# WenjieWWJ/FoodRec

Measured on NVIDIA B200. Metric: bpr_train_triples_per_sec, higher is better.
Workload: dtype f32

## Files before the change

foodrec_b200/csrc/api.cu:

```cuda
#include "ctx.h"

extern "C" int fr_abi_version(void) { return FR_ABI_VERSION; }

extern "C" int fr_create(const fr_config* cfg, fr_handle* out) {
  if (!cfg || !out) return FR_ERR_ARG;
  *out = nullptr;
  fr_ctx* h = new fr_ctx();
  *out = h;
  h->cfg = *cfg;
  const int D = cfg->embed_size;
  if (D <= 0 || D % 4 != 0 || D > 256) return fail(h, FR_ERR_ARG, "embed_size must be a multiple of 4 in (0,256], got %d", D);
  if (cfg->num_users <= 0 || cfg->num_items <= 0 || cfg->num_labels <= 0 || cfg->max_rows <= 0)
    return fail(h, FR_ERR_ARG, "num_users/num_items/num_labels/max_rows must be positive");
  if (cfg->learner < FR_SGD || cfg->learner > FR_ADAM) return fail(h, FR_ERR_ARG, "bad learner %d", cfg->learner);
  if (cfg->learner == FR_ADAM && cfg->adam_mode == FR_ADAM_LAZY_SERIES) {
    const double b1 = cfg->adam_beta1, b2 = cfg->adam_beta2;
    if (!(b1 >= 0.0 && b1 < 1.0 && b2 > 0.0 && b2 < 1.0)) return fail(h, FR_ERR_ARG, "adam betas must lie in [0,1) / (0,1)");
    double lead = 0.0, rem = 0.0, p1 = 1.0;
    for (int j = 1; j <= SERIES_WINDOW; ++j) {
      p1 *= b1;
      const double d = 1.0 - pow(b2, 0.5 * j);
      lead += p1;
      rem += p1 * pow(d, SERIES_TERMS) / (1.0 - d);
    }
// ... 1 lines not shown
      return fail(h, FR_ERR_UNSUPPORTED, "adam_mode LAZY_SERIES does not cover beta1=%g beta2=%g (tail %.1e, truncation %.1e): "
                  "use FR_ADAM_LAZY_EXACT", b1, b2, p1, lead > 0.0 ? rem / lead : 0.0);
  }
  int ndev = 0;
  cudaError_t e = cudaGetDeviceCount(&ndev);
  if (e != cudaSuccess || ndev == 0)
    return fail(h, FR_ERR_CUDA, "no CUDA device (%s); foodrec_b200 has no CPU fallback", cudaGetErrorString(e));
  FR_CUDA(h, cudaGetDevice(&h->device));
  cudaDeviceProp prop;
  FR_CUDA(h, cudaGetDeviceProperties(&prop, h->device));
  h->sm_count = prop.multiProcessorCount;
  h->l2_persist_max = (size_t)prop.persistingL2CacheMaxSize;
  h->l2_window_max = (size_t)prop.accessPolicyMaxWindowSize;
  if (getenv("FOODREC_NO_L2_PIN")) h->l2_persist_max = 0;
  if (getenv("FOODREC_DEBUG_L2"))
    fprintf(stderr, "foodrec_b200: L2 %d MB, persisting max %zu MB, access window max %zu MB\n", prop.l2CacheSize >> 20,
            h->l2_persist_max >> 20, h->l2_window_max >> 20);
  h->mc.D = D; h->mc.DV = D / 4; h->mc.L = cfg->num_labels;
  h->mc.a = cfg->high_level_score_coefficient;
  h->mc.oma = 1.0f - cfg->high_level_score_coefficient;
  h->mc.beta_1 = cfg->beta_1; h->mc.beta_2 = cfg->beta_2; h->mc.alpha = cfg->alpha;
  h->NV = h->mc.DV <= 32 ? 1 : 2;
  h->b1p = cfg->adam_beta1; h->b2p = cfg->adam_beta2;

  const size_t S = (size_t)cfg->max_rows, E = (size_t)(cfg->max_label_entries > 0 ? cfg->max_label_entries : 1);
  const size_t DV = h->mc.DV;
  int rc;
#define A(p, n) if ((rc = dalloc(h, &(p), (n)))) return rc
  A(h->ukeys, S); A(h->users_s, S); A(h->items_s, S); A(h->ws_row, S); A(h->g, S); A(h->scores, S); A(h->z, S * DV);
  if ((rc = alloc_sort(h, h->sortU, S))) return rc;
  if ((rc = alloc_sort(h, h->sortI, S))) return rc;
  if ((rc = alloc_sort(h, h->sortL, E))) return rc;
  h->fwd_grid_cap = h->sm_count * 4;
  A(h->part_loss, h->fwd_grid_cap); A(h->part_nrm, h->fwd_grid_cap); A(h->part_gcat, (size_t)h->fwd_grid_cap * 4 * DV);
  A(h->packed, 4 + 4 * (size_t)D + 5 * (size_t)cfg->num_labels * D);
  const size_t chS = S / 32 + 2, chE = E / 32 + 2;
  A(h->pieces_u, chS * 2 * 5 * DV); A(h->pieces_i, chS * 2 * DV); A(h->pieces_g, chE * 2 * 5 * DV);
  h->long_cap = (uint32_t)((chS > chE ? chS : chE) / FR_LONG_CHAIN + 2);
  A(h->long_list, h->long_cap);
  A(h->counts, S + 1); A(h->offs, S + 1); A(h->ent_key, E); A(h->ent_row, E); A(h->ent_coef, E); A(h->n_entries, 1);
  A(h->counters, 4); A(h->cat_pre, 4 * DV); A(h->mean_partials, 1024); A(h->out_internal, FR_OUT_COUNT);
  A(h->scan_tmp, S / 4096 + 2);
  h->lr_hist_cap = 1 << 16;
  A(h->lr_hist, (size_t)h->lr_hist_cap);
  A(h->cser, (size_t)h->lr_hist_cap * SERIES_TERMS);
#undef A
  FR_CUDA(h, cudaMemset(h->lr_hist, 0, (size_t)h->lr_hist_cap * sizeof(float)));
  FR_CUDA(h, cudaMemset(h->cser, 0, (size_t)h->lr_hist_cap * SERIES_TERMS * sizeof(double)));
  FR_CUDA(h, cudaMemset(h->out_internal, 0, FR_OUT_COUNT * sizeof(float)));
  return FR_OK;
}

extern "C" int64_t fr_launch_count(void) { return (int64_t)fr::g_launches; }

bool l2_window(fr_ctx* h, const void* ptr, size_t bytes, cudaAccessPolicyWindow* w) {
  if (!h->l2_persist_max || !h->l2_window_max || !bytes) return false;
  static bool limit_set = false;
  if (!limit_set) { cudaDeviceSetLimit(cudaLimitPersistingL2CacheSize, h->l2_persist_max); cudaGetLastError(); limit_set = true; }
  const size_t win = bytes < h->l2_window_max ? bytes : h->l2_window_max;
  w->base_ptr = const_cast<void*>(ptr);
  w->num_bytes = win;
  const double r = (double)h->l2_persist_max / (double)win;
  w->hitRatio = r >= 1.0 ? 1.0f : (float)r;
  w->hitProp = cudaAccessPropertyPersisting;
  w->missProp = cudaAccessPropertyNormal;
  return true;
}

extern "C" int fr_timing_enable(fr_handle h, int32_t enable) {
  if (!h) return FR_ERR_ARG;
  if (enable && h->tsets.empty()) {
    h->tsets.resize(32);
    for (auto& ts : h->tsets)
      for (auto& e : ts.ev) FR_CUDA(h, cudaEventCreate(&e));
  }
  h->timing = enable != 0;
  return FR_OK;
}

extern "C" int fr_timing_read(fr_handle h, double* ms_sum, int64_t* n_steps, int32_t reset) {
  if (!h || !ms_sum || !n_steps) return FR_ERR_ARG;
  for (auto& ts : h->tsets) timing_collect(h, ts);
  for (int i = 0; i < FR_T_COUNT; ++i) ms_sum[i] = h->t_sum[i];
  *n_steps = h->t_steps;
  if (reset) { for (auto& x : h->t_sum) x = 0.0; h->t_steps = 0; }
  return FR_OK;
}

extern "C" int fr_destroy(fr_handle h) {
  if (!h) return FR_OK;
  for (auto& ts : h->tsets) for (auto& e : ts.ev) cudaEventDestroy(e);
  catalog_free(h);
  for (void* p : h->allocs) cudaFree(p);
  if (h->stage) cudaFree(h->stage);
  for (auto& sl : h->feed) { if (sl.buf) cudaFree(sl.buf); if (sl.copied) cudaEventDestroy(sl.copied); if (sl.consumed) cudaEventDestroy(sl.consumed); }
  if (h->copy_stream) cudaStreamDestroy(h->copy_stream);
  if (h->aux_stream) { cudaStreamDestroy(h->aux_stream); cudaEventDestroy(h->aux_fork); cudaEventDestroy(h->aux_fork2); cudaEventDestroy(h->aux_join);
                       cudaStreamDestroy(h->aux2_stream); cudaEventDestroy(h->aux2_fork); cudaEventDestroy(h->aux2_join); }
  if (h->pieces_personal) cudaFree(h->pieces_personal);
  delete h;
  return FR_OK;
}

extern "C" const char* fr_last_error(fr_handle h) { return h ? h->err : "null handle"; }

extern "C" int fr_set_tables(fr_handle h, const fr_tables* t) {
// ... 551 lines not shown
```

foodrec_b200/csrc/common.cuh:

```cuda
#pragma once
#include <cuda_bf16.h>
#include <cuda_runtime.h>
#include <stdint.h>

#define FR_FULL 0xffffffffu
#define FR_WARPS_PER_BLOCK 8
#define FR_THREADS (FR_WARPS_PER_BLOCK * 32)

namespace fr {

__device__ __forceinline__ float warp_sum(float v) {
#pragma unroll
  for (int o = 16; o; o >>= 1) v += __shfl_xor_sync(FR_FULL, v, o);
  return v;
}
__device__ __forceinline__ double warp_sum_d(double v) {
#pragma unroll
  for (int o = 16; o; o >>= 1) v += __shfl_xor_sync(FR_FULL, v, o);
  return v;
}
__device__ __forceinline__ float4 f4zero() { return make_float4(0.f, 0.f, 0.f, 0.f); }
__device__ __forceinline__ float dot4(const float4 a, const float4 b) {
  return fmaf(a.w, b.w, fmaf(a.z, b.z, fmaf(a.y, b.y, a.x * b.x)));
}
__device__ __forceinline__ void fma4(float4& acc, const float s, const float4 v) {
  acc.x = fmaf(s, v.x, acc.x); acc.y = fmaf(s, v.y, acc.y);
  acc.z = fmaf(s, v.z, acc.z); acc.w = fmaf(s, v.w, acc.w);
}
__device__ __forceinline__ void mad4_rn(float4& acc, const float s, const float4 v) {
  acc.x = __fadd_rn(acc.x, __fmul_rn(s, v.x)); acc.y = __fadd_rn(acc.y, __fmul_rn(s, v.y));
  acc.z = __fadd_rn(acc.z, __fmul_rn(s, v.z)); acc.w = __fadd_rn(acc.w, __fmul_rn(s, v.w));
}
__device__ __forceinline__ float4 div4_rn(const float4 v, const float n) {
  return make_float4(__fdiv_rn(v.x, n), __fdiv_rn(v.y, n), __fdiv_rn(v.z, n), __fdiv_rn(v.w, n));
}
__device__ __forceinline__ float4 add4(const float4 a, const float4 b) {
  return make_float4(a.x + b.x, a.y + b.y, a.z + b.z, a.w + b.w);
}
__device__ __forceinline__ float4 scale4(const float s, const float4 v) {
  return make_float4(s * v.x, s * v.y, s * v.z, s * v.w);
}
__device__ __forceinline__ float4 shfl4(const float4 v, const int src) {
  return make_float4(__shfl_sync(FR_FULL, v.x, src), __shfl_sync(FR_FULL, v.y, src),
                     __shfl_sync(FR_FULL, v.z, src), __shfl_sync(FR_FULL, v.w, src));
}

__device__ __forceinline__ float4 ld_stream(const float4* p) {
  float4 r;
  asm volatile("ld.global.L1::no_allocate.v4.f32 {%0,%1,%2,%3}, [%4];"
               : "=f"(r.x), "=f"(r.y), "=f"(r.z), "=f"(r.w) : "l"(p));
  return r;
}
__device__ __forceinline__ void st_stream(float4* p, const float4 v) {
  asm volatile("st.global.L1::no_allocate.v4.f32 [%0], {%1,%2,%3,%4};"
               :: "l"(p), "f"(v.x), "f"(v.y), "f"(v.z), "f"(v.w) : "memory");
}

__device__ __forceinline__ void prefetch_l2_warp(const void* p, uint32_t bytes, int lane) {
#if defined(FR_PREFETCH_LINES)
  for (uint32_t o = (uint32_t)lane * 128u; o < bytes; o += 32u * 128u)
    asm volatile("prefetch.global.L2 [%0];" :: "l"(reinterpret_cast<const char*>(p) + o));
#else
  if (lane == 0) asm volatile("cp.async.bulk.prefetch.L2.global [%0], %1;" :: "l"(p), "r"(bytes) : "memory");
#endif
}

template <int NV>
__device__ __forceinline__ void load_row(float4 (&dst)[NV], const float4* row, int DV, int lane) {
#pragma unroll
  for (int k = 0; k < NV; ++k) {
    const int i = lane + 32 * k;
    dst[k] = (i < DV) ? ld_stream(row + i) : f4zero();
  }
}
template <int NV>
__device__ __forceinline__ void load_row_ro(float4 (&dst)[NV], const float4* __restrict__ row, int DV, int lane) {
#pragma unroll
  for (int k = 0; k < NV; ++k) {
    const int i = lane + 32 * k;
    dst[k] = (i < DV) ? __ldg(row + i) : f4zero();
  }
}
template <int NV>
__device__ __forceinline__ void load_row_cs(float4 (&dst)[NV], const float4* row, int DV, int lane) {
#pragma unroll
  for (int k = 0; k < NV; ++k) {
    const int i = lane + 32 * k;
    dst[k] = (i < DV) ? __ldcs(row + i) : f4zero();
  }
}
template <int NV>
__device__ __forceinline__ void store_row(float4* row, const float4 (&src)[NV], int DV, int lane) {
#pragma unroll
  for (int k = 0; k < NV; ++k) {
    const int i = lane + 32 * k;
    if (i < DV) st_stream(row + i, src[k]);
  }
}

template <bool BF> struct TabVec { using type = float4; };
template <> struct TabVec<true> { using type = uint2; };
template <bool BF>
__device__ __forceinline__ const typename TabVec<BF>::type* tab_at(const float4* base, size_t idx4) {
  return reinterpret_cast<const typename TabVec<BF>::type*>(base) + idx4;
}
template <bool BF>
__device__ __forceinline__ typename TabVec<BF>::type* tab_at(float4* base, size_t idx4) {
  return reinterpret_cast<typename TabVec<BF>::type*>(base) + idx4;
}
__device__ __forceinline__ float4 bf4_to_f4(const uint2 v) {
  return make_float4(__uint_as_float(v.x << 16), __uint_as_float(v.x & 0xffff0000u),
                     __uint_as_float(v.y << 16), __uint_as_float(v.y & 0xffff0000u));
}
__device__ __forceinline__ uint2 f4_to_bf4(const float4 v) {
  const __nv_bfloat162 a = __floats2bfloat162_rn(v.x, v.y), b = __floats2bfloat162_rn(v.z, v.w);
  uint2 r;
  r.x = *reinterpret_cast<const uint32_t*>(&a); r.y = *reinterpret_cast<const uint32_t*>(&b);
  return r;
// ... 97 lines not shown
```

foodrec_b200/csrc/eval.cu:

```cuda
#include "common.cuh"
#include "internal.h"

namespace fr {

template <int NV, class V>
__device__ __forceinline__ float score_pair(const float4 (&pr)[5][NV], const V* __restrict__ Rrow,
                                            const float4 m, const float4* sCat, int DV, int lane,
                                            float a, float oma) {
  float4 rr[NV], pcs[NV];
  load_row_ro_t<NV>(rr, Rrow, DV, lane);
  pooled_cat<NV>(pcs, sCat, m, DV, lane);
  float hs = 0.f, ls = 0.f;
#pragma unroll
  for (int k = 0; k < NV; ++k) {
    float4 zs;
    zs.x = m.x * pr[1][k].x + m.y * pr[2][k].x + m.z * pr[3][k].x + m.w * pr[4][k].x;
    zs.y = m.x * pr[1][k].y + m.y * pr[2][k].y + m.z * pr[3][k].y + m.w * pr[4][k].y;
    zs.z = m.x * pr[1][k].z + m.y * pr[2][k].z + m.z * pr[3][k].z + m.w * pr[4][k].z;
    zs.w = m.x * pr[1][k].w + m.y * pr[2][k].w + m.z * pr[3][k].w + m.w * pr[4][k].w;
    hs += dot4(pr[0][k], pcs[k]);
    ls += dot4(zs, rr[k]);
  }
  hs = warp_sum(hs); ls = warp_sum(ls);
  const float n = ((m.x + m.y) + m.z) + m.w;
// ... 3 lines not shown
template <int NV, bool BF>
__global__ void __launch_bounds__(FR_THREADS)
fwd_score_kernel(const float4* __restrict__ P, const float4* __restrict__ R, const float4* __restrict__ Cat,
                 int DV, const int32_t* __restrict__ users, const int32_t* __restrict__ items,
                 const float4* __restrict__ cats, int cats_by_item, int n, float a, float oma,
                 float* __restrict__ scores, const HealthBlend hb, uint32_t n_users, uint32_t n_items) {
  extern __shared__ float4 sCat[];
  for (int i = threadIdx.x; i < 4 * DV; i += blockDim.x) sCat[i] = Cat[i];
  __syncthreads();
  const int lane = threadIdx.x & 31;
  const int gw = blockIdx.x * FR_WARPS_PER_BLOCK + (threadIdx.x >> 5), nw = gridDim.x * FR_WARPS_PER_BLOCK;
  int cur_u = -1;
  float4 pr[5][NV];
  constexpr int RPW = 8;
  for (int blk = gw; blk * RPW < n; blk += nw) {
    for (int q = 0; q < RPW; ++q) {
      const int r = blk * RPW + q;
      if (r >= n) break;
      const int u = users[r];
      const int it = items[r];
      if ((uint32_t)u >= n_users || (uint32_t)it >= n_items) {
        if (lane == 0) scores[r] = __int_as_float(0x7fc00000);
        continue;
      }
      if (u != cur_u) {
#pragma unroll
        for (int s = 0; s < 5; ++s) load_row_ro_t<NV>(pr[s], tab_at<BF>(P, ((size_t)u * 5 + s) * DV), DV, lane);
        health_blend_rows<NV>(pr, hb, u, DV, lane);
        cur_u = u;
      }
      const float4 m = __ldg(cats + (cats_by_item ? it : r));
      const float s = score_pair<NV>(pr, tab_at<BF>(R, (size_t)it * DV), m, sCat, DV, lane, a, oma);
      if (lane == 0) scores[r] = s;
    }
  }
}

void launch_fwd_score(const ModelConsts& mc, const float4* P, const float4* R, const float4* Cat,
                      const int32_t* users, const int32_t* items, const float4* cats,
                      int cats_by_item, int n, float* scores, const HealthBlend& hb, const Launch& l,
                      int64_t n_users, int64_t n_items, int bf16) {
  if (n <= 0) return;
  int grid = (n + 8 * FR_WARPS_PER_BLOCK - 1) / (8 * FR_WARPS_PER_BLOCK);
  if (grid > l.sm_count * 8) grid = l.sm_count * 8;
  const size_t smem = (size_t)4 * mc.DV * sizeof(float4);
  ++g_launches;
#define FR_SCORE(NVV, BFF) fwd_score_kernel<NVV, BFF><<<grid, FR_THREADS, smem, l.st>>>(P, R, Cat, mc.DV, users, items, cats, cats_by_item, \
    n, mc.a, mc.oma, scores, hb, (uint32_t)n_users, (uint32_t)n_items)
  if (mc.DV <= 32) { if (bf16) FR_SCORE(1, true); else FR_SCORE(1, false); }
  else             { if (bf16) FR_SCORE(2, true); else FR_SCORE(2, false); }
#undef FR_SCORE
}

__device__ __forceinline__ void cp_async_vec(float4* dst, const float4* src) {
  const uint32_t d = (uint32_t)__cvta_generic_to_shared(dst);
  asm volatile("cp.async.cg.shared.global [%0], [%1], 16;" :: "r"(d), "l"(src) : "memory");
}
__device__ __forceinline__ void cp_async_vec(uint2* dst, const uint2* src) {
  const uint32_t d = (uint32_t)__cvta_generic_to_shared(dst);
  asm volatile("cp.async.ca.shared.global [%0], [%1], 8;" :: "r"(d), "l"(src) : "memory");
}
__device__ __forceinline__ void cp_async_commit() { asm volatile("cp.async.commit_group;" ::: "memory"); }
template <int N> __device__ __forceinline__ void cp_async_wait() { asm volatile("cp.async.wait_group %0;" :: "n"(N) : "memory"); }
__device__ __forceinline__ float4 ring_ld(const float4* p) { return *p; }
__device__ __forceinline__ float4 ring_ld(const uint2* p) { return bf4_to_f4(*p); }

constexpr int EV_WARPS = 4;
constexpr int EV_THREADS = EV_WARPS * 32;
constexpr int EV_CB = 8;
#ifndef FR_EV_GROUPS
#define FR_EV_GROUPS 2
#endif
#ifndef FR_EV_MINB
#define FR_EV_MINB 4
#endif
template <int NV> struct EvRing { static constexpr int GROUPS = FR_EV_GROUPS; };

template <int NV, int SLOTS, bool BF, bool EXACT>
__global__ void __launch_bounds__(EV_THREADS, NV == 1 ? FR_EV_MINB : (FR_EV_MINB > 3 ? 3 : FR_EV_MINB))
eval_sampled_kernel(const float4* __restrict__ P, const float4* __restrict__ R, const float4* __restrict__ Cat,
                    int DV, float a, float oma, const int32_t* __restrict__ users,
                    const int32_t* __restrict__ cand, const int32_t* __restrict__ n_cand, int n_users,
                    int stride, const float4* __restrict__ cand_cats, const float4* __restrict__ item_cats,
                    int K, int32_t* __restrict__ topk_ids, int32_t* __restrict__ gt_rank,
                    float* __restrict__ scores_out, const HealthBlend hb, uint32_t n_table_users, uint32_t n_items) {
  extern __shared__ float4 smem[];
  float4* sCat = smem;
  for (int i = threadIdx.x; i < 4 * DV; i += blockDim.x) sCat[i] = Cat[i];
  __syncthreads();
  const int lane = threadIdx.x & 31;
  float4* sM = smem + 4 * DV + (threadIdx.x >> 5) * (40 * SLOTS);
  uint32_t* sO = reinterpret_cast<uint32_t*>(sM + 32 * SLOTS);
  using V = typename TabVec<BF>::type;
  constexpr int GROUPS = EvRing<NV>::GROUPS;
  V* const ring = reinterpret_cast<V*>(smem + 4 * DV + EV_WARPS * (40 * SLOTS)) + ((threadIdx.x >> 5) * (GROUPS * EV_CB * NV) * 32 + lane);
  const int gw = blockIdx.x * EV_WARPS + (threadIdx.x >> 5), nw = gridDim.x * EV_WARPS;
  const typename TabVec<BF>::type* Rl = tab_at<BF>(R, 0) + lane;
  asm volatile("" : "+l"(Rl));
  constexpr int VB = (int)sizeof(typename TabVec<BF>::type);
  int un = 0, ncn = 0, idn[SLOTS];
  float4 pr[5][NV], mqn[SLOTS];
  auto fetch_ids = [&](int w2) {
    if (w2 < n_users) {
      un = users[w2]; ncn = n_cand[w2];
#pragma unroll
      for (int q = 0; q < SLOTS; ++q) {
        const int j = q * 32 + lane;
        idn[q] = j < stride ? cand[(size_t)w2 * stride + j] : -1;
      }
    }
  };
  auto fetch_rows = [&](int w2) {
    if (w2 >= n_users) return;
    if ((uint32_t)un < n_table_users) {
#pragma unroll
      for (int s = 0; s < 5; ++s) load_row_cs_t<NV>(pr[s], tab_at<BF>(P, ((size_t)un * 5 + s) * DV), DV, lane);
// ... 235 lines not shown
```

foodrec_b200/csrc/train.cuh:

```cuda
#pragma once
#include "internal.h"

namespace fr {

struct FwdParams {
  const float4 *P, *R, *cat;
  int DV, B;
  float Bnorm;
  const int32_t *users, *items;
  const float4* cats; int cats_by_item;
  const float* labels;
  float a, oma;
  float* g; float4* z; float* scores;
  float *part_loss, *part_nrm; float4* part_gcat;
  int lazy; const float4 *mP, *vP; const int32_t* lastP; OptConsts oc;
  int tab;
};

struct FinalizeParams {
  const float *part_loss, *part_nrm; const float4* part_gcat; int nblk;
  int DV; float inv_count_B;
  float B;
  float* packed;
  int do_reduce, do_apply;
  float4 *Cat, *s1Cat, *s2Cat;
  OptConsts oc; float clip;
  float* out; float* lr_hist;
};

struct SegCommon {
  const uint32_t* keys; const uint32_t* perm;
  const uint32_t* n_dev; uint32_t n_host;
  float4* pieces;
  uint32_t* uniq_counter;
  uint4* long_list;
  uint32_t* long_count; uint32_t long_cap;
  const float* only_if_scaled;
};
constexpr uint32_t FR_LONG_CHAIN = 16;

struct UserPolParams {
  float4 *P, *s1, *s2; int32_t* last;
  const float4 *R, *G; const float4* cat;
  const int32_t* items; const float* g; const float4* cats; int cats_by_item;
  const float* ws_row; const float* out;
  int group; ModelConsts mc; OptConsts oc;
  const float* user_labels; const int32_t *lab_off, *lab_idx; const int32_t* users;
  int tab;
};
struct FusedParams {
  float4 *P[2], *m[2], *v[2];
  int32_t* last;
  const float4 *R, *cat;
  const int32_t* items; const float4* cats; int cats_by_item;
  const float* labels;
  float a, oma, Bnorm;
  float* g; float4* z; float* scores;
  float *part_loss, *part_nrm; float4* part_gcat;
  ModelConsts mc; OptConsts oc;
};
int user_fused_grid(uint32_t n_rows, int sm_count);
void launch_user_fused(int NV, int group, const SegCommon& c, const FusedParams& p, int grid, const Launch& l);
void launch_user_commit(const uint32_t* keys, uint32_t n, int32_t* last, const float* out, int step, const Launch& l);
void launch_shadow_consolidate(int32_t* last, int64_t n_users, int rowDV, float4* P, float4* m, float4* v, const float4* Pa,
                               const float4* ma, const float4* va, const float* pred, const Launch& l);

struct ItemPolParams {
  float4 *R, *s1, *s2; int32_t* last;
  const float4* z; const float* g; const float* out;
  ModelConsts mc; OptConsts oc;
  int tab;
};
struct LabelPolParams {
  float4* G; const float4 *R, *cat;
  const uint32_t* ent_row; const float* ent_coef;
  const int32_t* items; const float4* cats; int cats_by_item;
  ModelConsts mc;
  int tab;
};

struct LabelEmitParams {
  int S, group, L; const int32_t* users;
  const float* user_labels; const int32_t *lab_off, *lab_idx;
  const float* ws_row;
  uint32_t* counts;
  const uint32_t* offs;
  uint32_t *ent_key, *ent_row; float* ent_coef; uint32_t cap;
  uint32_t* n_entries; float* out;
};

void launch_prep_rows(int mode, int B, const int32_t* users, const int32_t* items, const float* labels, const float* ws_in,
                      int64_t n_users, int64_t n_items, uint32_t* ukeys, float* ws_row, int32_t* users_s, int32_t* items_s,
                      float* flag, const Launch& l);
void launch_fwd_train(int NV, int group, const FwdParams& p, int grid, const Launch& l);
int fwd_train_grid(int B, int sm_count);
void launch_finalize(const FinalizeParams& p, const Launch& l);
void launch_user_pass(int NV, const SegCommon& c, const UserPolParams& p, const Launch& l);
void launch_personal_pass(int NV, const SegCommon& c, const UserPolParams& p, const Launch& l);
void launch_item_pass(int NV, const SegCommon& c, const ItemPolParams& p, const Launch& l);
void launch_label_pass(int NV, const SegCommon& c, const LabelPolParams& p, const Launch& l);
void launch_label_count(const LabelEmitParams& p, const Launch& l);
void launch_label_emit(const LabelEmitParams& p, const Launch& l);
void launch_adam_sweep(float4* var, float4* m, float4* v, int32_t* last, int64_t nrows, int rowDV,
                       const OptConsts& oc, int target_step, const Launch& l);
void launch_fill_i32(int32_t* p, int64_t n, int32_t v, const Launch& l);
void launch_series_update(double* cser, const float* lr_hist, int t, float b1, float b2, const Launch& l);
void launch_series_rebuild(double* cser, const float* lr_hist, int step, float b1, float b2, const Launch& l);
void launch_item_catchup(int NV, const uint32_t* keys, uint32_t n, float4* R, float4* m, float4* v,
                         int32_t* last, int DV, const OptConsts& oc, const Launch& l,
                         const uint32_t* n_dev = nullptr);
struct PeerPtrs { float4* dst[8]; int world, rank, cap; };
void launch_item_grad_pass(int NV, const SegCommon& c, const ItemPolParams& p, float4* gbuf, const PeerPtrs& peers, const Launch& l);

struct ShardPlanParams {
// ... 32 lines not shown
```

foodrec_b200/csrc/train_seg.cu:

```cuda
#include <cstdlib>

#include "optim.cuh"
#include "train.cuh"

namespace fr {

template <class Pol>
__global__ void __launch_bounds__(FR_THREADS)
seg_chunk_kernel(const SegCommon c, const Pol pol) {
  extern __shared__ float4 smem[];
  constexpr int NR = Pol::NR, NV = Pol::NV;
  const int DV = pol.DV();
  if (c.only_if_scaled && c.only_if_scaled[FR_OUT_SCALE] == 1.0f) return;
  if (pol.cat_src()) {
    for (int i = threadIdx.x; i < 4 * DV; i += blockDim.x) smem[i] = pol.cat_src()[i];
    __syncthreads();
  }
  const uint32_t n = c.n_dev ? min(*c.n_dev, c.n_host) : c.n_host;
  const uint32_t nchunks = (n + 31) >> 5;
  const int lane = threadIdx.x & 31;
  const uint32_t gw = blockIdx.x * FR_WARPS_PER_BLOCK + (threadIdx.x >> 5);
  const uint32_t nw = gridDim.x * FR_WARPS_PER_BLOCK;
  for (uint32_t chunk = gw; chunk < nchunks; chunk += nw) {
    const uint32_t base = chunk << 5;
// ... 740 lines not shown
  if (l.mid) cudaEventRecord(l.mid, l.st);
  seg_combine_kernel<Pol><<<grid, FR_THREADS, 0, l.st>>>(c, pol);
  g_launches += 2;
  launch_combine_long(c, pol, DV, l);
}

template <int NVV, int OPT>
struct FusedUserPol {
  static constexpr int NV = NVV;
  static constexpr int NR = 5;
  FusedParams p;
  struct State { float4 var[5][NVV], s1[5][NVV], s2[5][NVV]; int last, sh; };
  __device__ __forceinline__ int DV() const { return p.mc.DV; }
  __device__ __forceinline__ void load_state(State& st, uint32_t key, int lane) const {
    const int l = p.last[key];
    st.sh = (l >> 30) & 1; st.last = l & 0x3fffffff;
    const int DVv = p.mc.DV;
    const size_t base = (size_t)key * 5 * DVv;
    const float4 *Ps = p.P[st.sh] + base, *ms = p.m[st.sh] + base, *vs = p.v[st.sh] + base;
#pragma unroll
    for (int s = 0; s < 5; ++s)
#pragma unroll
      for (int k = 0; k < NV; ++k) {
        const int i = lane + 32 * k;
        const bool ok = i < DVv;
        st.var[s][k] = ok ? __ldcs(Ps + s * DVv + i) : f4zero();
        st.s1[s][k] = ok ? __ldcs(ms + s * DVv + i) : f4zero();
        st.s2[s][k] = ok ? __ldcs(vs + s * DVv + i) : f4zero();
      }
  }
  __device__ __forceinline__ void apply_to_other(State& st, uint32_t key, const float4 (&grad)[5][NV], int lane, bool caught) const {
    if (!caught) adam_catchup<OPT, 5 * NV>(&st.var[0][0], &st.s1[0][0], &st.s2[0][0], st.last, p.oc.step - 1, p.oc);
    const int DVv = p.mc.DV;
    const size_t base = (size_t)key * 5 * DVv;
    float4 *Pd = p.P[st.sh ^ 1] + base, *md = p.m[st.sh ^ 1] + base, *vd = p.v[st.sh ^ 1] + base;
#pragma unroll
    for (int s = 0; s < 5; ++s)
#pragma unroll
      for (int k = 0; k < NV; ++k) {
        const int i = lane + 32 * k;
        if (i >= DVv) continue;
        float4 var = st.var[s][k], a = st.s1[s][k], b = st.s2[s][k];
        const float4 g = grad[s][k];
        adam_touch(var.x, a.x, b.x, g.x, p.oc); adam_touch(var.y, a.y, b.y, g.y, p.oc);
        adam_touch(var.z, a.z, b.z, g.z, p.oc); adam_touch(var.w, a.w, b.w, g.w, p.oc);
        __stcs(Pd + s * DVv + i, var); __stcs(md + s * DVv + i, a); __stcs(vd + s * DVv + i, b);
      }
  }
  __device__ __forceinline__ void apply(State& st, uint32_t key, float4 (&acc)[5][NV], int lane) const {
    apply_to_other(st, key, acc, lane, false);
  }
};

template <int NV, int GROUP, int OPT>
__global__ void __launch_bounds__(FR_THREADS, NV == 1 ? 2 : 1)
user_fused_kernel(const SegCommon c, const FusedUserPol<NV, OPT> pol) {
  extern __shared__ float4 smem[];
  const FusedParams& p = pol.p;
  const int DV = p.mc.DV;
  float4* sCat = smem;
  float4* sgc = smem + 4 * DV;
  __shared__ float red_loss[FR_WARPS_PER_BLOCK], red_nrm[FR_WARPS_PER_BLOCK];
  for (int i = threadIdx.x; i < 4 * DV; i += blockDim.x) sCat[i] = p.cat[i];
  for (int i = threadIdx.x; i < FR_WARPS_PER_BLOCK * 4 * DV; i += blockDim.x) sgc[i] = f4zero();
  __syncthreads();
  const int lane = threadIdx.x & 31, warp = threadIdx.x >> 5;
  float4* mygc = sgc + warp * 4 * DV;
  const uint32_t n = c.n_host;
  const uint32_t nchunks = (n + 31) >> 5;
  const uint32_t gw = blockIdx.x * FR_WARPS_PER_BLOCK + warp, nw = gridDim.x * FR_WARPS_PER_BLOCK;
  const float a = p.a, oma = p.oma, Bf = p.Bnorm;
  float lossacc = 0.f, nrmacc = 0.f;
  for (uint32_t chunk = gw; chunk < nchunks; chunk += nw) {
    const uint32_t base = chunk << 5;
    const int cnt = (int)min(32u, n - base);
    const bool valid = lane < cnt;
    const uint32_t key = valid ? c.keys[base + lane] : 0xffffffffu;
    const uint32_t ent = valid ? c.perm[base + lane] : 0u;
    const uint32_t prevKey = base > 0 ? c.keys[base - 1] : 0u;
    const bool has_next = base + 32 < n;
    const uint32_t nextKey = has_next ? c.keys[base + 32] : 0u;
    int e_item = 0; float4 e_m = make_float4(1.f, 0.f, 0.f, 0.f); float e_y = 0.f; int e_last = 0;
    if (valid) {
      e_item = p.items[ent];
      e_m = __ldg(p.cats + (p.cats_by_item ? e_item : (int)ent));
      if (GROUP == 1) e_y = p.labels[ent];
      e_last = p.last[key];
    }
    const uint32_t up = __shfl_up_sync(FR_FULL, key, 1);
    const bool head = valid && (lane == 0 ? (base == 0 || prevKey != key) : (up != key));
    const uint32_t hm = __ballot_sync(FR_FULL, head);
    const uint32_t lastKey = __shfl_sync(FR_FULL, key, cnt - 1);
    const bool from_prev = !(hm & 1u);
    const bool to_next = has_next && nextKey == lastKey;
    if (c.uniq_counter && lane == 0) atomicAdd(c.uniq_counter, (uint32_t)__popc(hm));
    int e0 = 0;
    while (e0 < cnt) {
      const uint32_t rest = (e0 >= 31) ? 0u : (hm & ~((2u << e0) - 1u));
      const int e1 = rest ? (__ffs(rest) - 1) : cnt;
      const bool contained = ((e0 > 0) || !from_prev) && ((e1 < cnt) || !to_next);
      const uint32_t k = __shfl_sync(FR_FULL, key, e0);
      typename FusedUserPol<NV, OPT>::State st;
      {
        const int l = __shfl_sync(FR_FULL, e_last, e0);
        st.sh = (l >> 30) & 1; st.last = l & 0x3fffffff;
        const size_t ub = (size_t)k * 5 * DV;
        const float4 *Ps = p.P[st.sh] + ub, *ms = p.m[st.sh] + ub, *vs = p.v[st.sh] + ub;
#pragma unroll
        for (int s = 0; s < 5; ++s)
#pragma unroll
          for (int q = 0; q < NV; ++q) {
            const int i = lane + 32 * q;
            const bool ok = i < DV;
            st.var[s][q] = ok ? __ldcs(Ps + s * DV + i) : f4zero();
            st.s1[s][q] = ok ? __ldcs(ms + s * DV + i) : f4zero();
            st.s2[s][q] = ok ? __ldcs(vs + s * DV + i) : f4zero();
          }
      }
      float4 rr[GROUP][NV];
#pragma unroll
      for (int j = 0; j < GROUP; ++j)
        load_row_ro<NV>(rr[j], p.R + (size_t)__shfl_sync(FR_FULL, e_item, e0 + j) * DV, DV, lane);
      adam_catchup<OPT, 5 * NV>(&st.var[0][0], &st.s1[0][0], &st.s2[0][0], st.last, p.oc.step - 1, p.oc);
      float4 acc[5][NV];
#pragma unroll
      for (int s = 0; s < 5; ++s)
#pragma unroll
        for (int q = 0; q < NV; ++q) acc[s][q] = f4zero();
      for (int j0 = e0; j0 < e1; j0 += GROUP) {
        float4 pcn[GROUP][NV];
        float4 mm[GROUP]; float sc[GROUP], rnn[GROUP], nzq[GROUP], nRq[GROUP], npcq[GROUP];
        uint32_t row[GROUP];
#pragma unroll
        for (int j = 0; j < GROUP; ++j) {
          row[j] = __shfl_sync(FR_FULL, ent, j0 + j);
          mm[j] = shfl4(e_m, j0 + j);
        }
#pragma unroll
        for (int j = 0; j < GROUP; ++j) {
          const float4 m = mm[j];
          const float nn = ((m.x + m.y) + m.z) + m.w;
          const float rn = __frcp_rn(nn);
          float4 pcs[NV], zs[NV];
          pooled_cat<NV>(pcs, sCat, m, DV, lane);
          float hs = 0.f, ls = 0.f, nz = 0.f, nR = 0.f, npc = 0.f;
#pragma unroll
          for (int q = 0; q < NV; ++q) {
            zs[q].x = m.x * st.var[1][q].x + m.y * st.var[2][q].x + m.z * st.var[3][q].x + m.w * st.var[4][q].x;
            zs[q].y = m.x * st.var[1][q].y + m.y * st.var[2][q].y + m.z * st.var[3][q].y + m.w * st.var[4][q].y;
            zs[q].z = m.x * st.var[1][q].z + m.y * st.var[2][q].z + m.z * st.var[3][q].z + m.w * st.var[4][q].z;
            zs[q].w = m.x * st.var[1][q].w + m.y * st.var[2][q].w + m.z * st.var[3][q].w + m.w * st.var[4][q].w;
            hs += dot4(st.var[0][q], pcs[q]);
            ls += dot4(zs[q], rr[j][q]);
            nz += dot4(zs[q], zs[q]);
            if constexpr (GROUP == 1) { nR += dot4(rr[j][q], rr[j][q]); npc += dot4(pcs[q], pcs[q]); }
          }
          hs = warp_sum(hs); ls = warp_sum(ls);
          sc[j] = a * (hs * rn) + oma * (ls * rn);
          const float zc = oma * rn;
#pragma unroll
          for (int q = 0; q < NV; ++q) {
            const int i = lane + 32 * q;
            if (i < DV) __stcg(p.z + (size_t)row[j] * DV + i, scale4(zc, zs[q]));
            pcn[j][q] = scale4(rn, pcs[q]);
          }
          rnn[j] = rn;
          const float inv2 = rn * rn;
          nzq[j] = nz * inv2; nRq[j] = nR * inv2; npcq[j] = npc * inv2;
        }
        float gq[GROUP];
        if constexpr (GROUP == 1) {
          const float s = sc[0], y = __shfl_sync(FR_FULL, e_y, j0);
          const float e = expf(-fabsf(s));
          const float loss = fmaxf(s, 0.f) - s * y + log1pf(e);
          const float sig = s >= 0.f ? 1.f / (1.f + e) : e / (1.f + e);
          const float g = (sig - y) / Bf;
          const float4 m = mm[0];
          const float sumsq_m = m.x * m.x + m.y * m.y + m.z * m.z + m.w * m.w;
          const float nrm = g * g * (a * a * npcq[0] + oma * oma * (nRq[0] * sumsq_m + nzq[0]));
          const float ga = g * a, rn = rnn[0];
#pragma unroll
          for (int q = 0; q < NV; ++q) {
            const int i = lane + 32 * q;
            if (i < DV) {
              float4 t;
              t = mygc[i]; fma4(t, ga * (m.x * rn), st.var[0][q]); mygc[i] = t;
              t = mygc[DV + i]; fma4(t, ga * (m.y * rn), st.var[0][q]); mygc[DV + i] = t;
              t = mygc[2 * DV + i]; fma4(t, ga * (m.z * rn), st.var[0][q]); mygc[2 * DV + i] = t;
              t = mygc[3 * DV + i]; fma4(t, ga * (m.w * rn), st.var[0][q]); mygc[3 * DV + i] = t;
            }
          }
          lossacc += loss; nrmacc += nrm;
          gq[0] = g;
          if (lane == 0) { p.g[row[0]] = g; p.scores[row[0]] = s; }
        } else {
          const float s = sc[0] - sc[GROUP - 1];
          const float e = expf(-fabsf(s));
          const float loss = fmaxf(s, 0.f) - s + log1pf(e);
          const float sig = s >= 0.f ? 1.f / (1.f + e) : e / (1.f + e);
          const float h = (sig - 1.f) / Bf;
          const float4 m0 = mm[0], m1 = mm[GROUP - 1];
          const float4 w0 = scale4(rnn[0], m0), w1 = scale4(rnn[GROUP - 1], m1);
          float dq = 0.f;
#pragma unroll
          for (int q = 0; q < NV; ++q) {
            const float4 r0 = rr[0][q], r1 = rr[GROUP - 1][q];
            float4 d = make_float4(pcn[0][q].x - pcn[GROUP - 1][q].x, pcn[0][q].y - pcn[GROUP - 1][q].y,
                                   pcn[0][q].z - pcn[GROUP - 1][q].z, pcn[0][q].w - pcn[GROUP - 1][q].w);
            dq += a * a * dot4(d, d);
#pragma unroll
            for (int cc = 0; cc < 4; ++cc) {
              const float wa = comp(w0, cc), wb = comp(w1, cc);
              d = make_float4(wa * r0.x - wb * r1.x, wa * r0.y - wb * r1.y, wa * r0.z - wb * r1.z, wa * r0.w - wb * r1.w);
              dq += oma * oma * dot4(d, d);
            }
          }
          const float nrm = h * h * (dq + oma * oma * (nzq[0] + nzq[GROUP - 1]));
          const float ha = h * a;
#pragma unroll
          for (int q = 0; q < NV; ++q) {
            const int i = lane + 32 * q;
            if (i < DV) {
              float4 t;
              t = mygc[i]; fma4(t, ha * (w0.x - w1.x), st.var[0][q]); mygc[i] = t;
              t = mygc[DV + i]; fma4(t, ha * (w0.y - w1.y), st.var[0][q]); mygc[DV + i] = t;
              t = mygc[2 * DV + i]; fma4(t, ha * (w0.z - w1.z), st.var[0][q]); mygc[2 * DV + i] = t;
              t = mygc[3 * DV + i]; fma4(t, ha * (w0.w - w1.w), st.var[0][q]); mygc[3 * DV + i] = t;
            }
          }
          lossacc += loss; nrmacc += nrm;
          gq[0] = h; gq[GROUP - 1] = -h;
          if (lane == 0) {
            p.g[row[0]] = h; p.g[row[GROUP - 1]] = -h;
            p.scores[row[0]] = sc[0]; p.scores[row[GROUP - 1]] = sc[GROUP - 1];
          }
        }
#pragma unroll
        for (int j = 0; j < GROUP; ++j) {
          const float4 wj = scale4(rnn[j], mm[j]);
          const float ga = gq[j] * a, go = gq[j] * oma;
#pragma unroll
          for (int q = 0; q < NV; ++q) {
            mad4_rn(acc[0][q], ga, pcn[j][q]);
            mad4_rn(acc[1][q], go * wj.x, rr[j][q]); mad4_rn(acc[2][q], go * wj.y, rr[j][q]);
            mad4_rn(acc[3][q], go * wj.z, rr[j][q]); mad4_rn(acc[4][q], go * wj.w, rr[j][q]);
          }
        }
        if (j0 + GROUP < e1) {
#pragma unroll
          for (int j = 0; j < GROUP; ++j)
            load_row_ro<NV>(rr[j], p.R + (size_t)__shfl_sync(FR_FULL, e_item, j0 + GROUP + j) * DV, DV, lane);
        }
      }
      if (contained) {
        pol.apply_to_other(st, k, acc, lane, true);
      } else {
        float4* dst = c.pieces + ((size_t)chunk * 2 + (e0 == 0 ? 0 : 1)) * 5 * DV;
#pragma unroll
        for (int s = 0; s < 5; ++s)
#pragma unroll
          for (int q = 0; q < NV; ++q) {
            const int i = lane + 32 * q;
            if (i < DV) __stcg(dst + s * DV + i, acc[s][q]);
          }
      }
      e0 = e1;
    }
  }
  nrmacc = warp_sum(nrmacc);
  if (lane == 0) { red_loss[warp] = lossacc; red_nrm[warp] = nrmacc; }
  __syncthreads();
  for (int j = threadIdx.x; j < 4 * DV; j += blockDim.x) {
    float4 s = sgc[j];
#pragma unroll
    for (int w = 1; w < FR_WARPS_PER_BLOCK; ++w) s = add4(s, sgc[w * 4 * DV + j]);
    p.part_gcat[(size_t)blockIdx.x * 4 * DV + j] = s;
  }
  if (threadIdx.x == 0) {
    float l = 0.f, q = 0.f;
#pragma unroll
    for (int w = 0; w < FR_WARPS_PER_BLOCK; ++w) { l += red_loss[w]; q += red_nrm[w]; }
    p.part_loss[blockIdx.x] = l; p.part_nrm[blockIdx.x] = q;
  }
}

__global__ void __launch_bounds__(256)
user_commit_kernel(const uint32_t* __restrict__ keys, uint32_t n, int32_t* __restrict__ last, const float* __restrict__ out, int step) {
  if (out[FR_OUT_SCALE] != 1.0f) return;
  for (uint32_t i = blockIdx.x * blockDim.x + threadIdx.x; i < n; i += gridDim.x * blockDim.x) {
    const uint32_t k = keys[i];
    if (i == 0 || keys[i - 1] != k) {
      const int l = last[k];
      last[k] = step | ((l ^ (int)FR_SHADOW_BIT) & (int)FR_SHADOW_BIT);
    }
  }
}

__global__ void __launch_bounds__(FR_THREADS)
shadow_consolidate_kernel(int32_t* __restrict__ last, int64_t n_users, int rowDV, float4* __restrict__ P, float4* __restrict__ m,
                          float4* __restrict__ v, const float4* __restrict__ Pa, const float4* __restrict__ ma,
                          const float4* __restrict__ va, const float* __restrict__ pred) {
  if (pred && pred[FR_OUT_SCALE] == 1.0f) return;
  const int lane = threadIdx.x & 31;
  const int64_t gw = (int64_t)blockIdx.x * FR_WARPS_PER_BLOCK + (threadIdx.x >> 5), nw = (int64_t)gridDim.x * FR_WARPS_PER_BLOCK;
  for (int64_t u0 = gw * 32; u0 < n_users; u0 += nw * 32) {
    const int64_t u = u0 + lane;
    const int l = u < n_users ? last[u] : 0;
    uint32_t mask = __ballot_sync(FR_FULL, (l & (int)FR_SHADOW_BIT) != 0);
    if (l & (int)FR_SHADOW_BIT) last[u] = l & ~(int)FR_SHADOW_BIT;
    while (mask) {
      const int j = __ffs(mask) - 1;
      mask &= mask - 1;
      const size_t b = (size_t)(u0 + j) * rowDV;
      for (int i = lane; i < rowDV; i += 32) {
        __stcs(P + b + i, __ldcs(Pa + b + i)); __stcs(m + b + i, __ldcs(ma + b + i)); __stcs(v + b + i, __ldcs(va + b + i));
      }
    }
  }
}

void launch_shadow_consolidate(int32_t* last, int64_t n_users, int rowDV, float4* P, float4* m, float4* v, const float4* Pa,
                               const float4* ma, const float4* va, const float* pred, const Launch& l) {
  if (n_users <= 0) return;
  int64_t grid = (n_users + FR_THREADS - 1) / FR_THREADS;
  if (grid > (int64_t)l.sm_count * 8) grid = (int64_t)l.sm_count * 8;
  shadow_consolidate_kernel<<<(int)grid, FR_THREADS, 0, l.st>>>(last, n_users, rowDV, P, m, v, Pa, ma, va, pred);
  ++g_launches;
}

int user_fused_grid(uint32_t n_rows, int sm_count) {
  const uint32_t nchunks = (n_rows + 31) / 32;
  int grid = (int)((nchunks + FR_WARPS_PER_BLOCK - 1) / FR_WARPS_PER_BLOCK);
  static int per_sm = -1;
  if (per_sm < 0) { const char* e = getenv("FOODREC_FUSED_CTAS_PER_SM"); per_sm = e ? atoi(e) : 2; if (per_sm < 1 || per_sm > 4) per_sm = 2; }
  const int cap = sm_count * per_sm;
  if (grid > cap) grid = cap;
  return grid < 1 ? 1 : grid;
}

void launch_user_fused(int NV, int group, const SegCommon& c, const FusedParams& p, int grid, const Launch& l) {
  const int opt = opt_of(p.oc.learner, p.oc.adam_mode);
  const size_t smem = (size_t)(4 * p.mc.DV) * sizeof(float4) * (1 + FR_WARPS_PER_BLOCK);
  const uint32_t nchunks = (c.n_host + 31) / 32;
  int cgrid = (int)((nchunks + FR_WARPS_PER_BLOCK - 1) / FR_WARPS_PER_BLOCK);
  if (cgrid > l.sm_count * 16) cgrid = l.sm_count * 16;
#define FR_FUSED(NVV, GG, OO) do { FusedUserPol<NVV, OO> pol{p};                                            \
    user_fused_kernel<NVV, GG, OO><<<grid, FR_THREADS, smem, l.st>>>(c, pol);                                \
    if (l.mid) cudaEventRecord(l.mid, l.st);                                                                 \
    seg_combine_kernel<FusedUserPol<NVV, OO>><<<cgrid, FR_THREADS, 0, l.st>>>(c, pol); } while (0)
#define FR_FUSED_O(NVV, GG) do { if (opt == OPT_ADAM_EXACT) FR_FUSED(NVV, GG, OPT_ADAM_EXACT); else FR_FUSED(NVV, GG, OPT_ADAM_SERIES); } while (0)
  if (NV == 1) { if (group == 1) FR_FUSED_O(1, 1); else FR_FUSED_O(1, 2); }
  else         { if (group == 1) FR_FUSED_O(2, 1); else FR_FUSED_O(2, 2); }
#undef FR_FUSED_O
#undef FR_FUSED
  g_launches += 2;
}

void launch_user_commit(const uint32_t* keys, uint32_t n, int32_t* last, const float* out, int step, const Launch& l) {
  int grid = (int)((n + 255) / 256);
  if (grid > l.sm_count * 8) grid = l.sm_count * 8;
  if (grid < 1) grid = 1;
  user_commit_kernel<<<grid, 256, 0, l.st>>>(keys, n, last, out, step);
  ++g_launches;
}

#define FR_DISPATCH_NV_OPT(NVx, OPTx, ...)                                                  \
  do {                                                                                        \
    if ((NVx) == 1) {                                                                         \
      switch (OPTx) {                                                                         \
        case OPT_ADAM_DENSE:  { constexpr int NV_ = 1, OPT_ = OPT_ADAM_DENSE;  __VA_ARGS__ } break;  \
        case OPT_ADAM_EXACT:  { constexpr int NV_ = 1, OPT_ = OPT_ADAM_EXACT;  __VA_ARGS__ } break;  \
        case OPT_ADAM_SERIES: { constexpr int NV_ = 1, OPT_ = OPT_ADAM_SERIES; __VA_ARGS__ } break;  \
        default:              { constexpr int NV_ = 1, OPT_ = OPT_GENERIC;     __VA_ARGS__ } break;  \
      }                                                                                       \
    } else {                                                                                  \
      switch (OPTx) {                                                                         \
        case OPT_ADAM_DENSE:  { constexpr int NV_ = 2, OPT_ = OPT_ADAM_DENSE;  __VA_ARGS__ } break;  \
        case OPT_ADAM_EXACT:  { constexpr int NV_ = 2, OPT_ = OPT_ADAM_EXACT;  __VA_ARGS__ } break;  \
        case OPT_ADAM_SERIES: { constexpr int NV_ = 2, OPT_ = OPT_ADAM_SERIES; __VA_ARGS__ } break;  \
        default:              { constexpr int NV_ = 2, OPT_ = OPT_GENERIC;     __VA_ARGS__ } break;  \
      }                                                                                       \
    }                                                                                         \
  } while (0)

void launch_user_pass(int NV, const SegCommon& c, const UserPolParams& p, const Launch& l) {
  const int opt = opt_of(p.oc.learner, p.oc.adam_mode);
  if (p.tab != 0) {
    if (NV == 1) { if (p.tab == 1) { UserPol<1, OPT_GENERIC, 1> pol{p}; launch_seg(c, pol, p.mc.DV, true, l); }
                   else { UserPol<1, OPT_GENERIC, 2> pol{p}; launch_seg(c, pol, p.mc.DV, true, l); } }
    else         { if (p.tab == 1) { UserPol<2, OPT_GENERIC, 1> pol{p}; launch_seg(c, pol, p.mc.DV, true, l); }
                   else { UserPol<2, OPT_GENERIC, 2> pol{p}; launch_seg(c, pol, p.mc.DV, true, l); } }
    return;
  }
  FR_DISPATCH_NV_OPT(NV, opt, { UserPol<NV_, OPT_> pol{p}; launch_seg(c, pol, p.mc.DV, true, l); });
}
void launch_personal_pass(int NV, const SegCommon& c, const UserPolParams& p, const Launch& l) {
  if (NV == 1) { PersonalPol<1> pol{p}; launch_seg(c, pol, p.mc.DV, true, l); }
  else { PersonalPol<2> pol{p}; launch_seg(c, pol, p.mc.DV, true, l); }
}
// ... 81 lines not shown
```

Measured before the change: 204.2 million.

## Prefetch next user segment state via cp.async and double-buffer chunk metadata

The fused user kernel now stages the next segment's parameter, first-moment and second-moment rows into per-warp shared memory with cp.async while the current segment computes. It also double-buffers each chunk's keys, items, categories, labels and last-step stamps in shared memory, replacing warp shuffles with shared reads. The aim is to hide global load latency of the large per-user optimizer state. The cost is much more dynamic shared memory (raised via func attributes), which can lower occupancy, plus extra sync and a wait_group on every segment.

```diff
diff --git a/foodrec_b200/csrc/api.cu b/foodrec_b200/csrc/api.cu
--- a/foodrec_b200/csrc/api.cu
+++ b/foodrec_b200/csrc/api.cu
@@ -77,6 +77,14 @@
 }
 
 extern "C" int64_t fr_launch_count(void) { return (int64_t)fr::g_launches; }
+
+extern "C" int fr_user_fused_occupancy(int32_t D, int32_t group, int32_t* ctas_per_sm, int64_t* smem_bytes) {
+  if (D <= 0 || D % 4 != 0 || D > 256 || (group != 1 && group != 2) || !ctas_per_sm || !smem_bytes) return FR_ERR_ARG;
+  const int DV = D / 4, NV = DV <= 32 ? 1 : 2;
+  *smem_bytes = (int64_t)fr::user_fused_smem(NV, DV);
+  *ctas_per_sm = fr::user_fused_ctas_per_sm(NV, group, DV);
+  return *ctas_per_sm > 0 ? FR_OK : FR_ERR_CUDA;
+}
 
 bool l2_window(fr_ctx* h, const void* ptr, size_t bytes, cudaAccessPolicyWindow* w) {
   if (!h->l2_persist_max || !h->l2_window_max || !bytes) return false;
diff --git a/foodrec_b200/csrc/common.cuh b/foodrec_b200/csrc/common.cuh
--- a/foodrec_b200/csrc/common.cuh
+++ b/foodrec_b200/csrc/common.cuh
@@ -64,6 +64,17 @@
   if (lane == 0) asm volatile("cp.async.bulk.prefetch.L2.global [%0], %1;" :: "l"(p), "r"(bytes) : "memory");
 #endif
 }
+
+__device__ __forceinline__ void cp_async_vec(float4* dst, const float4* src) {
+  const uint32_t d = (uint32_t)__cvta_generic_to_shared(dst);
+  asm volatile("cp.async.cg.shared.global [%0], [%1], 16;" :: "r"(d), "l"(src) : "memory");
+}
+__device__ __forceinline__ void cp_async_vec(uint2* dst, const uint2* src) {
+  const uint32_t d = (uint32_t)__cvta_generic_to_shared(dst);
+  asm volatile("cp.async.ca.shared.global [%0], [%1], 8;" :: "r"(d), "l"(src) : "memory");
+}
+__device__ __forceinline__ void cp_async_commit() { asm volatile("cp.async.commit_group;" ::: "memory"); }
+template <int N> __device__ __forceinline__ void cp_async_wait() { asm volatile("cp.async.wait_group %0;" :: "n"(N) : "memory"); }
 
 template <int NV>
 __device__ __forceinline__ void load_row(float4 (&dst)[NV], const float4* row, int DV, int lane) {
diff --git a/foodrec_b200/csrc/eval.cu b/foodrec_b200/csrc/eval.cu
--- a/foodrec_b200/csrc/eval.cu
+++ b/foodrec_b200/csrc/eval.cu
@@ -79,16 +79,6 @@
 #undef FR_SCORE
 }
 
-__device__ __forceinline__ void cp_async_vec(float4* dst, const float4* src) {
-  const uint32_t d = (uint32_t)__cvta_generic_to_shared(dst);
-  asm volatile("cp.async.cg.shared.global [%0], [%1], 16;" :: "r"(d), "l"(src) : "memory");
-}
-__device__ __forceinline__ void cp_async_vec(uint2* dst, const uint2* src) {
-  const uint32_t d = (uint32_t)__cvta_generic_to_shared(dst);
-  asm volatile("cp.async.ca.shared.global [%0], [%1], 8;" :: "r"(d), "l"(src) : "memory");
-}
-__device__ __forceinline__ void cp_async_commit() { asm volatile("cp.async.commit_group;" ::: "memory"); }
-template <int N> __device__ __forceinline__ void cp_async_wait() { asm volatile("cp.async.wait_group %0;" :: "n"(N) : "memory"); }
 __device__ __forceinline__ float4 ring_ld(const float4* p) { return *p; }
 __device__ __forceinline__ float4 ring_ld(const uint2* p) { return bf4_to_f4(*p); }
 
diff --git a/foodrec_b200/csrc/train.cuh b/foodrec_b200/csrc/train.cuh
--- a/foodrec_b200/csrc/train.cuh
+++ b/foodrec_b200/csrc/train.cuh
@@ -60,6 +60,8 @@
   ModelConsts mc; OptConsts oc;
 };
 int user_fused_grid(uint32_t n_rows, int sm_count);
+size_t user_fused_smem(int NV, int DV);
+int user_fused_ctas_per_sm(int NV, int group, int DV);
 void launch_user_fused(int NV, int group, const SegCommon& c, const FusedParams& p, int grid, const Launch& l);
 void launch_user_commit(const uint32_t* keys, uint32_t n, int32_t* last, const float* out, int step, const Launch& l);
 void launch_shadow_consolidate(int32_t* last, int64_t n_users, int rowDV, float4* P, float4* m, float4* v, const float4* Pa,
diff --git a/foodrec_b200/csrc/train_seg.cu b/foodrec_b200/csrc/train_seg.cu
--- a/foodrec_b200/csrc/train_seg.cu
+++ b/foodrec_b200/csrc/train_seg.cu
@@ -816,76 +816,129 @@
   }
 };
 
+struct FusedChunkSlot { int4 id[32]; float4 m[32]; uint4 x[32]; };
+
+template <int GROUP>
+__device__ __forceinline__ void fused_load_chunk(FusedChunkSlot* s, const SegCommon& c, const FusedParams& p, uint32_t chunk,
+                                                 uint32_t nchunks, int lane) {
+  __syncwarp();
+  const uint32_t n = c.n_host, base = chunk << 5;
+  const bool valid = chunk < nchunks && base + lane < n;
+  const uint32_t key = valid ? c.keys[base + lane] : 0xffffffffu;
+  const uint32_t ent = valid ? c.perm[base + lane] : 0u;
+  const uint32_t prevKey = (chunk < nchunks && base > 0) ? c.keys[base - 1] : 0u;
+  const uint32_t nextKey = (chunk < nchunks && base + 32 < n) ? c.keys[base + 32] : 0u;
+  int item = 0, last = 0; float4 m = make_float4(1.f, 0.f, 0.f, 0.f); float y = 0.f;
+  if (valid) {
+    item = p.items[ent];
+    m = __ldg(p.cats + (p.cats_by_item ? item : (int)ent));
+    if (GROUP == 1) y = p.labels[ent];
+    last = p.last[key];
+  }
+  s->id[lane] = make_int4((int)key, (int)ent, item, last);
+  s->m[lane] = m;
+  s->x[lane] = make_uint4(prevKey, nextKey, __float_as_uint(y), 0u);
+  __syncwarp();
+}
+
+constexpr int FUSED_STAGE_SLOTS = 15;
+
+template <int NV>
+__device__ __forceinline__ void fused_stage_issue(float4* buf, const FusedParams& p, uint32_t key, int stamp, int DV, int lane) {
+  const int sh = (stamp >> 30) & 1;
+  const size_t ub = (size_t)key * 5 * DV;
+  const float4* src[3] = {p.P[sh] + ub, p.m[sh] + ub, p.v[sh] + ub};
+#pragma unroll
+  for (int r = 0; r < 3; ++r)
+#pragma unroll
+    for (int s = 0; s < 5; ++s)
+#pragma unroll
+      for (int q = 0; q < NV; ++q) {
+        const int i = lane + 32 * q;
+        if (i < DV) cp_async_vec(buf + ((r * 5 + s) * NV + q) * 32 + lane, src[r] + s * DV + i);
+      }
+  cp_async_commit();
+}
+
+size_t user_fused_smem(int NV, int DV) {
+  return ((size_t)4 * DV * (1 + FR_WARPS_PER_BLOCK) + (size_t)FR_WARPS_PER_BLOCK * FUSED_STAGE_SLOTS * NV * 32) * sizeof(float4) +
+         FR_WARPS_PER_BLOCK * 2 * sizeof(FusedChunkSlot);
+}
+
 template <int NV, int GROUP, int OPT>
 __global__ void __launch_bounds__(FR_THREADS, NV == 1 ? 2 : 1)
 user_fused_kernel(const SegCommon c, const FusedUserPol<NV, OPT> pol) {
   extern __shared__ float4 smem[];
+  constexpr int SLOTS = FUSED_STAGE_SLOTS;
   const FusedParams& p = pol.p;
   const int DV = p.mc.DV;
   float4* sCat = smem;
   float4* sgc = smem + 4 * DV;
+  float4* sstage = sgc + FR_WARPS_PER_BLOCK * 4 * DV;
+  FusedChunkSlot* schunk = reinterpret_cast<FusedChunkSlot*>(sstage + FR_WARPS_PER_BLOCK * SLOTS * NV * 32);
   __shared__ float red_loss[FR_WARPS_PER_BLOCK], red_nrm[FR_WARPS_PER_BLOCK];
   for (int i = threadIdx.x; i < 4 * DV; i += blockDim.x) sCat[i] = p.cat[i];
   for (int i = threadIdx.x; i < FR_WARPS_PER_BLOCK * 4 * DV; i += blockDim.x) sgc[i] = f4zero();
   __syncthreads();
   const int lane = threadIdx.x & 31, warp = threadIdx.x >> 5;
   float4* mygc = sgc + warp * 4 * DV;
+  float4* stg = sstage + warp * SLOTS * NV * 32;
+  FusedChunkSlot* cs = schunk + 2 * warp;
+  int ph = 0;
   const uint32_t n = c.n_host;
   const uint32_t nchunks = (n + 31) >> 5;
   const uint32_t gw = blockIdx.x * FR_WARPS_PER_BLOCK + warp, nw = gridDim.x * FR_WARPS_PER_BLOCK;
   const float a = p.a, oma = p.oma, Bf = p.Bnorm;
   float lossacc = 0.f, nrmacc = 0.f;
+  fused_load_chunk<GROUP>(cs, c, p, gw, nchunks, lane);
+  if (gw < nchunks) fused_stage_issue<NV>(stg, p, (uint32_t)cs->id[0].x, cs->id[0].w, DV, lane);
   for (uint32_t chunk = gw; chunk < nchunks; chunk += nw) {
     const uint32_t base = chunk << 5;
     const int cnt = (int)min(32u, n - base);
     const bool valid = lane < cnt;
-    const uint32_t key = valid ? c.keys[base + lane] : 0xffffffffu;
-    const uint32_t ent = valid ? c.perm[base + lane] : 0u;
-    const uint32_t prevKey = base > 0 ? c.keys[base - 1] : 0u;
+    const FusedChunkSlot* cur = cs + ph;
+    FusedChunkSlot* nx = cs + (ph ^ 1);
+    ph ^= 1;
+    const uint32_t key = (uint32_t)cur->id[lane].x;
+    const uint2 cx = make_uint2(cur->x[lane].x, cur->x[lane].y);
+    fused_load_chunk<GROUP>(nx, c, p, chunk + nw, nchunks, lane);
+    const bool more = chunk + nw < nchunks;
     const bool has_next = base + 32 < n;
-    const uint32_t nextKey = has_next ? c.keys[base + 32] : 0u;
-    int e_item = 0; float4 e_m = make_float4(1.f, 0.f, 0.f, 0.f); float e_y = 0.f; int e_last = 0;
-    if (valid) {
-      e_item = p.items[ent];
-      e_m = __ldg(p.cats + (p.cats_by_item ? e_item : (int)ent));
-      if (GROUP == 1) e_y = p.labels[ent];
-      e_last = p.last[key];
-    }
     const uint32_t up = __shfl_up_sync(FR_FULL, key, 1);
-    const bool head = valid && (lane == 0 ? (base == 0 || prevKey != key) : (up != key));
+    const bool head = valid && (lane == 0 ? (base == 0 || cx.x != key) : (up != key));
     const uint32_t hm = __ballot_sync(FR_FULL, head);
     const uint32_t lastKey = __shfl_sync(FR_FULL, key, cnt - 1);
     const bool from_prev = !(hm & 1u);
-    const bool to_next = has_next && nextKey == lastKey;
+    const bool to_next = has_next && cx.y == lastKey;
     if (c.uniq_counter && lane == 0) atomicAdd(c.uniq_counter, (uint32_t)__popc(hm));
     int e0 = 0;
     while (e0 < cnt) {
       const uint32_t rest = (e0 >= 31) ? 0u : (hm & ~((2u << e0) - 1u));
       const int e1 = rest ? (__ffs(rest) - 1) : cnt;
       const bool contained = ((e0 > 0) || !from_prev) && ((e1 < cnt) || !to_next);
-      const uint32_t k = __shfl_sync(FR_FULL, key, e0);
+      const uint32_t k = (uint32_t)cur->id[e0].x;
       typename FusedUserPol<NV, OPT>::State st;
       {
-        const int l = __shfl_sync(FR_FULL, e_last, e0);
+        const int l = cur->id[e0].w;
         st.sh = (l >> 30) & 1; st.last = l & 0x3fffffff;
-        const size_t ub = (size_t)k * 5 * DV;
-        const float4 *Ps = p.P[st.sh] + ub, *ms = p.m[st.sh] + ub, *vs = p.v[st.sh] + ub;
+        cp_async_wait<0>();
 #pragma unroll
         for (int s = 0; s < 5; ++s)
 #pragma unroll
           for (int q = 0; q < NV; ++q) {
-            const int i = lane + 32 * q;
-            const bool ok = i < DV;
-            st.var[s][q] = ok ? __ldcs(Ps + s * DV + i) : f4zero();
-            st.s1[s][q] = ok ? __ldcs(ms + s * DV + i) : f4zero();
-            st.s2[s][q] = ok ? __ldcs(vs + s * DV + i) : f4zero();
+            const bool ok = lane + 32 * q < DV;
+            st.var[s][q] = ok ? stg[(s * NV + q) * 32 + lane] : f4zero();
+            st.s1[s][q] = ok ? stg[((5 + s) * NV + q) * 32 + lane] : f4zero();
+            st.s2[s][q] = ok ? stg[((10 + s) * NV + q) * 32 + lane] : f4zero();
           }
       }
       float4 rr[GROUP][NV];
 #pragma unroll
       for (int j = 0; j < GROUP; ++j)
-        load_row_ro<NV>(rr[j], p.R + (size_t)__shfl_sync(FR_FULL, e_item, e0 + j) * DV, DV, lane);
+        load_row_ro<NV>(rr[j], p.R + (size_t)cur->id[(e0 + j) & 31].z * DV, DV, lane);
       adam_catchup<OPT, 5 * NV>(&st.var[0][0], &st.s1[0][0], &st.s2[0][0], st.last, p.oc.step - 1, p.oc);
+      if (e1 < cnt) fused_stage_issue<NV>(stg, p, (uint32_t)cur->id[e1].x, cur->id[e1].w, DV, lane);
+      else if (more) fused_stage_issue<NV>(stg, p, (uint32_t)nx->id[0].x, nx->id[0].w, DV, lane);
       float4 acc[5][NV];
 #pragma unroll
       for (int s = 0; s < 5; ++s)
@@ -897,8 +950,8 @@
         uint32_t row[GROUP];
 #pragma unroll
         for (int j = 0; j < GROUP; ++j) {
-          row[j] = __shfl_sync(FR_FULL, ent, j0 + j);
-          mm[j] = shfl4(e_m, j0 + j);
+          row[j] = (uint32_t)cur->id[(j0 + j) & 31].y;
+          mm[j] = cur->m[(j0 + j) & 31];
         }
 #pragma unroll
         for (int j = 0; j < GROUP; ++j) {
@@ -934,7 +987,7 @@
         }
         float gq[GROUP];
         if constexpr (GROUP == 1) {
-          const float s = sc[0], y = __shfl_sync(FR_FULL, e_y, j0);
+          const float s = sc[0], y = __uint_as_float(cur->x[j0 & 31].z);
           const float e = expf(-fabsf(s));
           const float loss = fmaxf(s, 0.f) - s * y + log1pf(e);
           const float sig = s >= 0.f ? 1.f / (1.f + e) : e / (1.f + e);
@@ -1013,7 +1066,7 @@
         if (j0 + GROUP < e1) {
 #pragma unroll
           for (int j = 0; j < GROUP; ++j)
-            load_row_ro<NV>(rr[j], p.R + (size_t)__shfl_sync(FR_FULL, e_item, j0 + GROUP + j) * DV, DV, lane);
+            load_row_ro<NV>(rr[j], p.R + (size_t)cur->id[(j0 + GROUP + j) & 31].z * DV, DV, lane);
         }
       }
       if (contained) {
@@ -1102,13 +1155,34 @@
   return grid < 1 ? 1 : grid;
 }
 
+template <int NV, int GROUP, int OPT>
+static cudaError_t user_fused_configure(size_t smem) {
+  cudaError_t e = cudaFuncSetAttribute(user_fused_kernel<NV, GROUP, OPT>, cudaFuncAttributeMaxDynamicSharedMemorySize, (int)smem);
+  if (e == cudaSuccess)
+    e = cudaFuncSetAttribute(user_fused_kernel<NV, GROUP, OPT>, cudaFuncAttributePreferredSharedMemoryCarveout,
+                             (int)cudaSharedmemCarveoutMaxShared);
+  return e;
+}
+
+int user_fused_ctas_per_sm(int NV, int group, int DV) {
+  const size_t smem = user_fused_smem(NV, DV);
+  int per_sm = 0;
+#define FR_FUSED_OCC(NVV, GG) do { if (user_fused_configure<NVV, GG, OPT_ADAM_SERIES>(smem) == cudaSuccess)              \
+    cudaOccupancyMaxActiveBlocksPerMultiprocessor(&per_sm, user_fused_kernel<NVV, GG, OPT_ADAM_SERIES>, FR_THREADS, smem); } while (0)
+  if (NV == 1) { if (group == 1) FR_FUSED_OCC(1, 1); else FR_FUSED_OCC(1, 2); }
+  else         { if (group == 1) FR_FUSED_OCC(2, 1); else FR_FUSED_OCC(2, 2); }
+#undef FR_FUSED_OCC
+  return per_sm;
+}
+
 void launch_user_fused(int NV, int group, const SegCommon& c, const FusedParams& p, int grid, const Launch& l) {
   const int opt = opt_of(p.oc.learner, p.oc.adam_mode);
-  const size_t smem = (size_t)(4 * p.mc.DV) * sizeof(float4) * (1 + FR_WARPS_PER_BLOCK);
+  const size_t smem = user_fused_smem(NV, p.mc.DV);
   const uint32_t nchunks = (c.n_host + 31) / 32;
   int cgrid = (int)((nchunks + FR_WARPS_PER_BLOCK - 1) / FR_WARPS_PER_BLOCK);
   if (cgrid > l.sm_count * 16) cgrid = l.sm_count * 16;
 #define FR_FUSED(NVV, GG, OO) do { FusedUserPol<NVV, OO> pol{p};                                            \
+    user_fused_configure<NVV, GG, OO>(smem);                                                                 \
     user_fused_kernel<NVV, GG, OO><<<grid, FR_THREADS, smem, l.st>>>(c, pol);                                \
     if (l.mid) cudaEventRecord(l.mid, l.st);                                                                 \
     seg_combine_kernel<FusedUserPol<NVV, OO>><<<cgrid, FR_THREADS, 0, l.st>>>(c, pol); } while (0)
```

New measurement: 208.7 million, median of 6. 1.02x the previous value.
